# brson/synth2

Measured on AMD Instinct MI355X. Metric: voice-samples/sec (mono) at 64k voices per GPU, 48 kHz, 1024-frame buffers, higher is better.
Workload: dtype f32

## Files before the change

include/s2r.h:

```cpp
#ifndef S2R_H
#define S2R_H
#include <stddef.h>
#include <stdint.h>

#ifdef __cplusplus
extern "C" {
#endif

#define S2R_ABI_VERSION 4

typedef enum {
    S2R_OK = 0,
    S2R_ERR_INVALID = -1,
    S2R_ERR_NO_DEVICE = -2,
    S2R_ERR_HIP = -3,
    S2R_ERR_PATCH_SYNTAX = -4,
    S2R_ERR_PATCH_RANGE = -5,
    S2R_ERR_TOO_MANY_FRAMES = -6,
    S2R_ERR_OFFSET_OVERFLOW = -7,
    S2R_ERR_OUT_OF_MEMORY = -8
} s2r_status;

typedef enum { S2R_OSC_SQUARE = 0, S2R_OSC_SAW = 1, S2R_OSC_TRIANGLE = 2, S2R_OSC_SINE = 3,
               S2R_OSC_DPW_SAW = 4, S2R_OSC_DPW_SQUARE = 5, S2R_OSC_DPW_TRIANGLE = 6 } s2r_osc_kind;
// ... 197 lines not shown

typedef void (*s2r_voice_log_fn)(void *user, uint32_t voice_index, uint8_t note);
int s2r_set_voice_log(s2r_synth *s, s2r_voice_log_fn fn, void *user);

uint32_t s2r_abi_version(void);
const char *s2r_build_id(void);
uint32_t s2r_shard_voices(const s2r_synth *s);
uint32_t s2r_block_voices(const s2r_synth *s);
uint32_t s2r_device_count(const s2r_synth *s);
uint64_t s2r_double_release_count(const s2r_synth *s);
int s2r_set_low_latency(s2r_synth *s, int enabled);
int s2r_low_latency_active(const s2r_synth *s);
#define S2R_EXCHANGE_HANDLE_BYTES 64
int s2r_exchange_create(s2r_synth *s, uint32_t n_ranks, void *handle_out, size_t handle_bytes);
int s2r_exchange_attach(s2r_synth *s, uint32_t rank, uint32_t n_ranks, const void *handle, size_t handle_bytes);
int s2r_set_resident(s2r_synth *s, int enabled);
int s2r_resident_active(const s2r_synth *s);
int s2r_quiesce(s2r_synth *s);
int s2r_set_timing(s2r_synth *s, int enabled);
int s2r_set_flat_shortcut(s2r_synth *s, int enabled);
int s2r_set_coeff_stream(s2r_synth *s, int enabled);
int s2r_set_uniform_window(s2r_synth *s, int enabled);
int s2r_uniform_window_chunks(s2r_synth *s, uint64_t *chunks);
float s2r_last_render_ms(s2r_synth *s);
const char *s2r_last_error(const s2r_synth *s);
const char *s2r_status_string(int status);


#define S2R_STREAM_CHARS_PER_SAMPLE 18u
#define S2R_STREAM_FRAMES 4096u
#define S2R_STREAM_RATE_HZ 32000u
size_t s2r_stream_frame_json(const float *samples, size_t n, char *out, size_t cap);

int s2r_parse_patch_text(const char *text, size_t len, s2r_patch *out, char *err_buf, size_t err_cap);

float s2r_voice_pan(float pan, float key_spread, uint8_t note);
void s2r_pan_gains(float p, float *gl, float *gr);

float s2r_voice_gain(float level, float velocity_sens, float velocity);

void s2r_fader_gains(float pan, float w, float fader, float pan_shift, float *gl, float *gr);

float s2r_send_gain(float g, float send);

typedef struct s2r_voice_pool s2r_voice_pool;
s2r_voice_pool *s2r_voice_pool_create(uint32_t total_voices);
// ... 14 lines not shown
```

synth2_amd/csrc/s2r_device.h:

```cpp
#pragma once
#include <hip/hip_runtime_api.h>
#include <stdint.h>
#include "s2r.h"

#define S2R_VF_STARTED 1u
#define S2R_VF_RELEASED 2u

struct S2rEnv {
    float A;
    float D;
    float S;
    float R;
    float sus_off;
    float slope_att;
    float slope_dec;
    float slope_rel;
};

struct S2rVoiceArrays {
    float *pitch;
    uint32_t *offset;
    uint32_t *release;
    uint32_t *flags;
    float *phase;
// ... 76 lines not shown
    int32_t fast_div_sr;
    int32_t no_flat_shortcut;
    uint32_t frames;
    uint32_t n_voices;
    uint32_t frames_stride;
    uint32_t super_frames;
    S2rVoiceArrays v;
    float *block_partials;
    float *direct_out;
    int32_t direct_stereo;
    S2rDone done;
    float *per_voice;
    const float *sin_table;
    const float *noise_tab;
    S2rTabRef tab;
    const S2rTimedEvent *tev;
    int32_t *voice_ev_head;
    unsigned long long *stamps;
    unsigned long long *timeline;
    uint32_t tl_slot;
    uint32_t uw_frames;
    const S2rBankEntry *bank;
    uint32_t bank_size;
    const uint32_t *ov_heads_counter;
    uint32_t ov_heads_target;
    uint32_t *ov_render_counter;
    uint32_t *ov_fail;
    const S2rTimedEvent *tev_src;
    S2rTimedEvent *tev_copy;
    const uint32_t *slices;
    uint32_t *arrive;
    uint32_t arrive_target;
    S2rMixTail mt;
    uint32_t *uw_count;
};
#define S2R_UW_FRAMES 1024u
#define S2R_UW_PLANES 4u
#define S2R_UW_MIN_RUN 3u

struct S2rVoiceEvent {
    uint32_t voice;
    uint32_t flags;
    float pitch;
    uint32_t seed;
};
#define S2R_EV_RESTART 1u
#define S2R_EV_RELEASE 2u
#define S2R_EV_PROGRAM_SHIFT 16

struct S2rTimedEvent {
    uint32_t voice;
    uint32_t frame;
    uint32_t flags;
    float pitch;
    uint32_t seed;
    int32_t next;
    uint32_t program;
    uint32_t _pad;
// ... 210 lines not shown
```

synth2_amd/csrc/s2r_host.cpp:

```cpp
#include <hip/hip_runtime.h>
#include <algorithm>
#include <cmath>
#include <cstdarg>
#include <cstdio>
#include <cstdlib>
#include <cstring>
#include <ctime>
#include <atomic>
#include <memory>
#include <new>
#include <string>
#include <vector>

#include "s2r.h"
#include "s2r_device.h"
#include "s2r_math.h"
#include "s2r_patch.h"
#include "s2r_post.h"
#include "s2r_rules.h"
#include "s2r_voices.h"

namespace {

constexpr int kEventSlots = 4;
// ... 211 lines not shown
        }
    } mixer;
    unsigned gains_dirty = kGainsAll;
    float *gains_host = nullptr, *gains_dev = nullptr;
    hipEvent_t gains_sent = nullptr;
    float *pan_rows = nullptr;
    uint32_t pan_slice = 0;
    float *pan_partials = nullptr;
    std::vector<hipEvent_t> pan_ev;
    size_t pan_ev_used = 0;
    float pan_mix_ms = -1.0f;
    char *bus_gains_host = nullptr, *bus_gains_dev = nullptr;
    hipEvent_t bus_gains_sent = nullptr;
    float *bus_partials = nullptr;
    float *bus_out = nullptr, *bus_out_dev = nullptr;
    float bus_mix_ms = -1.0f;
    bool bus_dev_ramped = false;
    S2rPostChain post;
    float pitch_table[256];
    hipEvent_t t0 = nullptr, t1 = nullptr;
    bool timing = false, timed = false, no_flat_shortcut = false;
    uint64_t double_release = 0;
    bool uniform_window = true;
    uint32_t *uw_count_dev = nullptr;
    s2r_voice_log_fn voice_log = nullptr;
    void *voice_log_user = nullptr;
    bool broken = false;
    std::string err = "";
};


namespace {

int set_err(s2r_synth *s, int code, const char *fmt, ...) {
    if (s) {
        char buf[512];
        va_list ap; va_start(ap, fmt); vsnprintf(buf, sizeof buf, fmt, ap); va_end(ap);
        s->err = buf;
    }
    return code;
}

#define S2R_TRY(call) do { const int rc_t_ = (call); if (rc_t_ != S2R_OK) return rc_t_; } while (0)
#define S2R_QUIESCE(s) S2R_TRY(quiesce(s))
int resident_stop(s2r_synth *s);
int pool_stop(s2r_synth *s);
// ... 278 lines not shown
    p.noise_level = s->bank[0].noise;
    p.lpf_freq = s->bank[0].lpf_freq;
    p.amt_osc = s->bank[0].mod_env_to_osc_freq;
    p.amt_lpf = s->bank[0].mod_env_to_lpf_freq;
    p.lpf_kind = s->bank[0].lpf_kind;
    p.lpf_damping = s->bank[0].lpf_kind >= S2R_FILT_BP2 ? s->bank[0].lpf_q : s->bank[0].lpf_damping;
    p.amp = resolve_env(s->bank[0].amp_env, sample_rate);
    p.mod = resolve_env(s->bank[0].mod_env, sample_rate);
    p.sr = (float)sample_rate;
    p.rcp_sr = 1.0f / p.sr;
    p.fast_div_sr = (fast_div_rate(sample_rate) && s->bank[0].lpf_freq >= 0x1p-30f && s->bank[0].lpf_freq <= 0x1p30f) ? 1 : 0;
    p.no_flat_shortcut = s->no_flat_shortcut ? 1 : 0;
    p.frames = (uint32_t)frames;
    p.n_voices = s->shard_voices;
    p.frames_stride = partials_stride(s->cfg.max_frames);
    p.v = s->v;
    p.block_partials = s->block_partials;
    p.per_voice = nullptr;
    p.sin_table = s->sin_dev;
    { static const bool off = [] { const char *e = std::getenv("S2R_NOISE_TAB"); return e && e[0] == '0'; }();
      p.noise_tab = off ? nullptr : s->noise_dev; }
    p.bank = s->bank_dev;
    p.bank_size = (uint32_t)s->bank.size();
    p.uw_count = s->uniform_window ? s->uw_count_dev : nullptr;
    return p;
}

int ensure_bank(s2r_synth *s, uint32_t sample_rate, hipStream_t stream, bool *bank_kernel_out) {
    bool bank_kernel = s->bank.size() > 1;
    for (const s2r_patch &pt : s->bank) if (pt.osc_kind > S2R_OSC_SINE) bank_kernel = true;
    if (bank_kernel && (s->bank_dirty || s->bank_rate != sample_rate)) {
        std::vector<S2rBankEntry> host(s->bank.size());
        std::vector<S2rTabBuild> builds(s->bank.size());
        size_t tab_floats = 0;
        const float srf = (float)sample_rate;
        for (size_t k = 0; k < s->bank.size(); k++) {
            const s2r_patch &pt = s->bank[k];
            S2rBankEntry &e = host[k];
            std::memset(&e, 0, sizeof e);
            e.osc_kind = pt.osc_kind; e.osc_gain = pt.osc_gain; e.noise_level = pt.noise; e.lpf_freq = pt.lpf_freq;
            e.amt_osc = pt.mod_env_to_osc_freq; e.amt_lpf = pt.mod_env_to_lpf_freq; e.lpf_kind = pt.lpf_kind;
            e.lpf_shape = pt.lpf_kind >= S2R_FILT_BP2 ? pt.lpf_q : pt.lpf_damping;
            e.amp = resolve_env(pt.amp_env, sample_rate);
            e.mod = resolve_env(pt.mod_env, sample_rate);
            S2rTabBuild &b = builds[k];
            b = S2rTabBuild{};
            if (s->use_tab && !s->no_flat_shortcut && plan_tables(e.mod, b) && tab_floats + (size_t)b.plane * 4u <= ((size_t)1 << 28)) {
// ... 1246 lines not shown
            CREATE_HIP(hipMalloc((void **)&s->partials2[1], (size_t)s->n_blocks * partials_stride(cfg->max_frames) * sizeof(float)));
            CREATE_HIP(hipMalloc((void **)&s->heads2[1], pv * sizeof(int32_t)));
            CREATE_HIP(hipMemsetAsync(s->heads2[1], 0xff, pv * sizeof(int32_t), s->stream));
            CREATE_HIP(hipMalloc((void **)&s->tevcopy2[1], (size_t)s->tev_capacity * sizeof(S2rTimedEvent)));
            CREATE_HIP(hipMalloc((void **)&s->ov_words, sizeof(S2rOverlapWords)));
            CREATE_HIP(hipMemsetAsync(s->ov_words, 0, sizeof(S2rOverlapWords), s->stream));
            s->ov_enabled = true;
        }
    }
    CREATE_HIP(hipEventCreate(&s->t0));
    CREATE_HIP(hipEventCreate(&s->t1));
    {
        float table[1024];
        build_sin_table(table);
        if (crc32_bytes(table, sizeof table) != kSinTableCrc) {
            fprintf(stderr, "libs2r: regenerated SIN_TABLE does not match the reference table (CRC mismatch)\n");
            release_all(s);
            return S2R_ERR_INVALID;
        }
        CREATE_HIP(hipMalloc((void **)&s->sin_dev, sizeof table));
        CREATE_HIP(hipMemcpy(s->sin_dev, table, sizeof table, hipMemcpyHostToDevice));
        CREATE_HIP(hipMalloc((void **)&s->noise_dev, 65536 * sizeof(float)));
        CREATE_HIP(s2r_launch_noise_table(s->noise_dev, s->stream));
        CREATE_HIP(hipMalloc((void **)&s->uw_count_dev, sizeof(uint32_t)));
        CREATE_HIP(hipMemsetAsync(s->uw_count_dev, 0, sizeof(uint32_t), s->stream));
    }
    CREATE_HIP(hipStreamSynchronize(s->stream));
#undef CREATE_HIP
    *out = s;
    return S2R_OK;
}


int s2r_create(const s2r_config *cfg, s2r_synth **out) {
    if (!cfg || !out || cfg->struct_size != sizeof(s2r_config)) return S2R_ERR_INVALID;
    *out = nullptr;
    if (cfg->n_devices <= 1) {
        s2r_config one = *cfg;
        if (cfg->n_devices == 1) one.device = cfg->devices[0];
        one.n_devices = 0;
        return create_single(&one, nullptr, nullptr, out);
    }
    const uint32_t n = cfg->n_devices;
    const uint32_t bv = cfg->block_voices ? cfg->block_voices : 256u;
    if (n > S2R_MAX_DEVICES || cfg->total_voices == 0 || cfg->max_frames == 0 || cfg->reserved0 != 0) return S2R_ERR_INVALID;
    if (cfg->shard_begin || cfg->shard_voices || cfg->shard_index || cfg->shard_count > 1 || cfg->mix_groups > 1) return S2R_ERR_INVALID;
    if (bv < 64 || bv > 1024 || (bv & 63u) || cfg->total_voices % ((uint64_t)n * bv)) return S2R_ERR_INVALID;
    if (cfg->shard_interleave && ((cfg->shard_interleave & 15u) || bv % cfg->shard_interleave)) return S2R_ERR_INVALID;
// ... 1099 lines not shown
}

uint32_t s2r_shard_voices(const s2r_synth *s) { return s ? s->shard_voices : 0; }
uint32_t s2r_block_voices(const s2r_synth *s) { return s ? s->block_voices : 0; }
uint32_t s2r_device_count(const s2r_synth *s) { return s ? (s->kids.empty() ? 1u : (uint32_t)s->kids.size()) : 0; }
uint64_t s2r_double_release_count(const s2r_synth *s) { return s ? s->double_release : 0; }

int s2r_set_flat_shortcut(s2r_synth *s, int enabled) {
    if (!s) return S2R_ERR_INVALID;
    S2R_QUIESCE(s);
    s->no_flat_shortcut = enabled == 0;
    for (s2r_synth *kid : s->kids) kid->no_flat_shortcut = s->no_flat_shortcut;
    return S2R_OK;
}

int s2r_set_uniform_window(s2r_synth *s, int enabled) {
    if (!s) return S2R_ERR_INVALID;
    S2R_QUIESCE(s);
    s->uniform_window = enabled != 0;
    for (s2r_synth *kid : s->kids) kid->uniform_window = s->uniform_window;
    return S2R_OK;
}

int s2r_uniform_window_chunks(s2r_synth *s, uint64_t *chunks) {
    if (!s || !chunks) return S2R_ERR_INVALID;
    S2R_QUIESCE(s);
    uint64_t total = 0;
    auto one = [&](s2r_synth *h) -> int {
        if (!h->uw_count_dev) return S2R_OK;
        uint32_t n = 0;
        S2R_HIP(s, hipSetDevice(h->device));
        S2R_HIP(s, hipDeviceSynchronize());
        S2R_HIP(s, hipMemcpy(&n, h->uw_count_dev, sizeof n, hipMemcpyDeviceToHost));
        total += n;
        return S2R_OK;
    };
    if (s->kids.empty()) { S2R_TRY(one(s)); }
    else for (s2r_synth *kid : s->kids) { S2R_TRY(one(kid)); }
    *chunks = total;
    return S2R_OK;
}

int s2r_set_coeff_stream(s2r_synth *s, int enabled) {
    if (!s) return S2R_ERR_INVALID;
    S2R_QUIESCE(s);
    s->use_tab = enabled != 0;
    s->use_arg_events = enabled != 2 && enabled != 4;
    s->bank_dirty = true;
    for (s2r_synth *kid : s->kids) { kid->use_tab = s->use_tab; kid->use_arg_events = s->use_arg_events; kid->bank_dirty = true; }
    return S2R_OK;
}

int s2r_set_low_latency(s2r_synth *s, int enabled) {
    if (!s) return S2R_ERR_INVALID;
    if (s->parent || !s->kids.empty()) return set_err(s, S2R_ERR_INVALID, "s2r_set_low_latency takes a single-device handle");
    S2R_QUIESCE(s);
    if (enabled && !s->res_host) {
        S2R_HIP(s, hipSetDevice(s->device));
        S2R_HIP(s, hipHostMalloc((void **)&s->res_host, 64 * sizeof(uint32_t), kHostPolled));
        std::memset(s->res_host, 0, 64 * sizeof(uint32_t));
        S2R_HIP(s, hipHostGetDevicePointer((void **)&s->res_dev, s->res_host, 0));
        s->res_cmd = s->res_host; s->res_cmd_dev = s->res_dev; s->res_cmd_vram = false;
        S2R_HIP(s, hipHostMalloc((void **)&s->res_gran, S2R_RES_GRANULE_FRAMES * sizeof(unsigned long long), kHostPolled));
        std::memset(s->res_gran, 0, S2R_RES_GRANULE_FRAMES * sizeof(unsigned long long));
// ... 205 lines not shown
```

synth2_amd/csrc/s2r_render_onepole.inc:

```
#include "s2r_kern_common.h"

namespace {

template <int OSC, bool FM, int MODE, int MAXT, bool UWK = false>
__device__ __forceinline__ void render_fill(const S2rRenderArgs &a, const FillCtl &ctl) {
    const S2rRenderParams &p = a.p;
    constexpr bool PV = MODE == 1;
    constexpr bool TEV = MODE == 2;
    const uint32_t kSuper = p.super_frames;
    __shared__ uint64_t sT[S2R_EXP2F_N];
    __shared__ __attribute__((aligned(8))) float sSin[OSC == S2R_OSC_SINE ? 2048 : 2];
    extern __shared__ __attribute__((aligned(16))) float s_dyn[];
    __shared__ uint32_t s_word;

    const uint32_t tid = threadIdx.x;
    const uint32_t lane = tid & 63u, wave = tid >> 6, n_waves = blockDim.x >> 6;
    constexpr uint32_t VW = 64;
    constexpr uint32_t GW = VW / 16;
    const uint32_t n_groups = n_waves * GW;
    float *const sW = s_dyn;
    constexpr uint32_t kTile = kChunk * kTileRow;
    const uint32_t sw_floats = s2r_sw_buffers(p.frames, kSuper) * n_groups * kSuper;
    float *const tile = s_dyn + sw_floats + wave * kTile;
    float *const wave_scratch = s_dyn + sw_floats + n_waves * kTile + wave * (64u + (UWK ? S2R_UW_PLANES * p.uw_frames : 0u));
    uint32_t uw_chunks = 0;
    const uint32_t tile_lds = (uint32_t)__builtin_amdgcn_readfirstlane((int)(uint32_t)(uintptr_t)tile);
    const uint32_t vi = blockIdx.x * blockDim.x + tid;
#if defined(S2R_STAMPS)
    uint32_t stamp_k = 0;
    auto stamp = [&](uint32_t slot) { if (p.stamps && lane == 0 && slot < 16u) p.stamps[(size_t)(vi >> 6) * 16u + slot] = __builtin_amdgcn_s_memtime(); };
    stamp(0);
#else
    auto stamp = [&](uint32_t) {};
    uint32_t stamp_k = 0; (void)stamp_k;
#endif
    uint32_t dbg_events = 0, dbg_dense = 0, dbg_general = 0, dbg_runs = 0, dbg_runchunks = 0;
    unsigned long long dbg_t_dense = 0, dbg_t_run = 0;
    unsigned long long dbg_t_top = 0, dbg_t_sel = 0; (void)dbg_t_top; (void)dbg_t_sel;
    unsigned long long dbg_t_pick1 = 0, dbg_t_casc = 0; (void)dbg_t_pick1; (void)dbg_t_casc;
    (void)dbg_events; (void)dbg_dense; (void)dbg_general; (void)dbg_runs; (void)dbg_runchunks; (void)dbg_t_dense; (void)dbg_t_run;
#if defined(S2R_STAMPS)
#define S2R_DBG_NOW() __builtin_amdgcn_s_memtime()
#else
#define S2R_DBG_NOW() 0ull
#endif

    tl_mark(p.timeline, p.tl_slot, 0);
    if (tid < S2R_EXP2F_N) sT[tid] = c_exp2f_table[tid];
    if (OSC == S2R_OSC_SINE)
        for (uint32_t i = tid; i < 1024u; i += blockDim.x) { sSin[2u * i] = p.sin_table[(i + 1023u) & 1023u]; sSin[2u * i + 1u] = p.sin_table[i]; }

    apply_arg_events(p, ctl.n_events, ctl.ev, vi, lane);

    const bool in_range = vi < p.n_voices;
    const bool ovh = TEV && (ctl.fused || ctl.ov_heads_counter != nullptr);
    if (TEV && ctl.fused) { fused_heads(ctl); stamp(7); }
    else if (ovh) {
        if (tid == 0) { const bool ok = ov_wait(ctl.ov_heads_counter, ctl.ov_heads_target); if (!ok) ov_raise(ctl.fail, 1u); s_word = ok ? 1u : 0u; }
        __syncthreads();
        if (s_word == 0u) {
            float *row = ctl.partials + (size_t)blockIdx.x * p.frames_stride;
            for (uint32_t f = 4u * tid; f < p.frames_stride && f < ((ctl.frames + 3u) & ~3u); f += 4u * blockDim.x) ov_store4(row + f, (f4){0.0f, 0.0f, 0.0f, 0.0f});
// ... 51 lines not shown
        while (ev_idx >= 0 && !(ev_next.flags & S2R_EV_RESTART)) {
            const uint32_t rel = r.offset + ev_next.frame;
            const bool base_ok = r.offset <= (1u << 24) || r.offset >= 0u - ctl.frames;
            if (!(base_ok && rel <= (1u << 24))) break;
            if ((ev_next.flags & S2R_EV_RELEASE) && live && !r.released) {
                r.released = true;
                r.release_u = rel;
                took_release = true;
            }
            ev_dirty = true;
            ev_idx = ev_next.next;
            ev_frame = 0xffffffffu;
            if (ev_idx >= 0) { ev_next = tev_at(ev_idx); ev_frame = ev_next.frame; }
        }
    };
    if (TEV) take_releases();
    r.seed_rot = (seed << 5) | (seed >> 27);

    const float rel_f = r.released ? (float)r.release_u : 4294967296.0f;
    r.ro_a = __builtin_fmaxf(rel_f, p.amp.sus_off); r.end_a = r.ro_a + p.amp.R;
    r.ro_m = __builtin_fmaxf(rel_f, p.mod.sus_off); r.end_m = r.ro_m + p.mod.R;

    OscK k_const = make_osck<OSC>(p.sr / (1.0f * r.pitch));
    uint32_t seed_now = seed;

    EnvRun ea = env_stage_at(p.amp, r.ro_a, r.end_a, (float)r.offset);
    EnvRun em = env_stage_at(p.mod, r.ro_m, r.end_m, (float)r.offset);
    float thr_min = __builtin_fminf(ea.s3, em.s3);
    FlatCache fc;
    fc.xc = 0.0f; fc.k = k_const;

    __syncthreads();
    const bool have_tab = p.tab.base != nullptr && !p.no_flat_shortcut;
    FlatConsts fcc = (have_tab && (!FM || p.tab.fm_plane != 0u)) ? flat_consts_from_tables<OSC, FM>(p, r.pitch) : make_flat_consts<OSC, FM>(p, r.pitch, sT);
    fc = refresh_flat<OSC, FM>(fcc, em, fc);

    const bool wave_live = __ballot(live || ev_idx >= 0) != 0ull;
    bool wave_events = TEV && __ballot(ev_idx >= 0) != 0ull;
    const uint32_t x16_frames = ctl.frames & ~(uint32_t)(kChunk - 1);
    const bool fast_ok = __ballot(!(r.phase >= 0.0f && r.phase < 1.0f)) == 0ull &&
        (FM || __ballot(!(k_const.period >= 0x1p-126f && k_const.period < __builtin_inff())) == 0ull);
    const size_t pv_base = (size_t)vi * ctl.frames;
    float *bp = ctl.partials + (size_t)blockIdx.x * p.frames_stride;
    uint32_t buf = 0;

    auto reduce_chunk = [&](uint32_t f_base, uint32_t n_frames) {
        const uint32_t f = lane & 15u, grp = lane >> 4;
// ... 23 lines not shown
        w_aflat = __ballot(live && ea.s0 != 0.0f) == 0ull;
        classify_uniform();
    };
    auto reclassify = [&]() {
        reclassify_stages();
        w_aligned = p.noise_tab != nullptr && __ballot(((r.offset | r.seed_rot) & 15u) != 0u) == 0ull;
        w_small = __ballot(r.offset + ctl.frames > (1u << 24)) == 0ull;
    };
    reclassify();
    stamp(1);

    auto apply_events_lane = [&](uint32_t fpos) -> bool {
        bool restarted = false, released_now = false;
        took_release = false;
        while (ev_frame == fpos) {
            const S2rTimedEvent e = ev_next;
            if (e.flags & S2R_EV_RESTART) {
                r.pitch = e.pitch;
                r.offset = 0u - fpos;
                r.release_u = 0u;
                r.released = (e.flags & S2R_EV_RELEASE) != 0u;
                r.phase = 0.0f; r.last = 0.0f;
                const S2rTimedEvent er = tev_at(ev_idx);
                seed_now = er.seed;
                r.seed_rot = (seed_now << 5) | (seed_now >> 27);
                program_now = er.program;
                live = true; ev_restart = true; restarted = true;
                k_const = make_osck<OSC>(p.sr / (1.0f * r.pitch));
            } else if ((e.flags & S2R_EV_RELEASE) && live && !r.released) {
                r.released = true;
                r.release_u = r.offset + fpos;
                released_now = true;
            }
            ev_dirty = true;
            ev_idx = e.next;
            ev_frame = 0xffffffffu;
            if (ev_idx >= 0) { ev_next = tev_at(ev_idx); ev_frame = ev_next.frame; }
            take_releases();
        }
        const float rf = r.released ? (float)r.release_u : 4294967296.0f;
        r.ro_a = __builtin_fmaxf(rf, p.amp.sus_off); r.end_a = r.ro_a + p.amp.R;
        r.ro_m = __builtin_fmaxf(rf, p.mod.sus_off); r.end_m = r.ro_m + p.mod.R;
        const float t0 = (float)(r.offset + fpos);
        if (restarted) {
            if (FM) {
                const FlatConsts n = (have_tab && p.tab.fm_plane != 0u) ? flat_consts_from_tables<OSC, FM>(p, r.pitch) : make_flat_consts<OSC, FM>(p, r.pitch, sT);
                fcc.k_s = n.k_s; fcc.k_0 = n.k_0;
            }
// ... 141 lines not shown
                            const bool hit = ev_frame == fnext;
                            if (__ballot((hit && !plain) || !((float)(onext + (kChunk - 1u)) < thr_min)) != 0ull) break;
                            pend_rel = hit ? onext : pend_rel;
                            ev_frame = hit ? 0xffffffffu : ev_frame;
                            if ((c16 & 0x30u) == 0x30u) {
                                const uint64_t pending = __ballot(ev_frame != 0xffffffffu);
                                if (pending == 0ull) { idle_exit = true; break; }
                                if (__builtin_popcountll(pending) <= 4) {
                                    const uint32_t nxt = wave_min_u32(ev_frame);
                                    if (((nxt - fnext) >> 4) > 8u) { idle_exit = true; break; }
                                }
                            }
                        }
                    }
                    commit_plain();
                    wave_events = __ballot(ev_idx >= 0) != 0ull;
                    dense_stay = wave_events && !idle_exit && !inside && c16 >= n_x16;
                    dbg_t_dense += S2R_DBG_NOW() - dbg_td0;
                    reclassify();
                    if (c16 >= n_x16) break;
                    if (!inside) { c16 -= kChunk; continue; }
                }
                const unsigned long long dbg_ts0 = S2R_DBG_NOW();
                const uint32_t o_chunk = r.offset + sc0 + c16;
                if (fast_ok) {
                    const uint32_t left = (n_x16 - c16) / kChunk;
                    auto clear_for = [&](uint32_t n) {
                        bool bad = !((float)(o_chunk + n * kChunk - 1u) < thr_min);
                        if (TEV) bad = bad || ev_frame < sc0 + c16 + n * kChunk;
                        return __ballot(bad) == 0ull;
                    };
                    auto pick_run = [&]() -> uint32_t {
                        const float q = ((thr_min - (float)o_chunk) + 1.0f) * 0.0625f;
                        float nf = __builtin_ceilf(q) - 1.0f;
                        nf = __builtin_fminf(__builtin_fmaxf(nf, 0.0f), (float)left);
                        uint32_t n = (uint32_t)nf;
                        if (TEV) { const uint32_t ne = (ev_frame - (sc0 + c16)) >> 4; n = ne < n ? ne : n; }
                        n = wave_min_u32(n);
                        if (n == 0u) return 0u;
                        if (clear_for(n)) return n;
                        return (n > 1u && clear_for(1u)) ? 1u : 0u;
                    };
                    {
                        const float t0 = (float)o_chunk;
                        if (__ballot(!(t0 < thr_min)) != 0ull) {
                            end_of_release(t0);
                            thr_min = __builtin_fminf(ea.s3, em.s3);
                            if (!(t0 < thr_min)) {
                                ea = env_stage_at(p.amp, r.ro_a, r.end_a, t0);
                                em = env_stage_at(p.mod, r.ro_m, r.end_m, t0);
                                thr_min = __builtin_fminf(ea.s3, em.s3);
                            }
                            fc = refresh_flat<OSC, FM>(fcc, em, fc);
                            reclassify_stages();
                        }
                    }
                    const unsigned long long dbg_ts1 = S2R_DBG_NOW();
                    dbg_t_casc += dbg_ts1 - dbg_ts0;
                    uint32_t run = pick_run();
                    dbg_t_pick1 += S2R_DBG_NOW() - dbg_ts1;
                    bool flat = false, tab_ok = false, offs_small = false;
                    if (run) {
                        run = (uint32_t)__builtin_amdgcn_readfirstlane((int)run);
                        offs_small = w_small || __ballot(o_chunk + run * kChunk > (1u << 24)) == 0ull;
                        flat = w_flat;
                        tab_ok = !flat && have_tab && offs_small;
                        if (FM && !flat && !tab_ok) run = 0;
                        if (FM && !flat && __ballot(live && !(p.sr >= r.pitch * 0x1p-115f)) != 0ull) run = 0;
                    }
                    if (run) {
                        ++dbg_runs; dbg_runchunks += run;
                        const unsigned long long dbg_tr0 = S2R_DBG_NOW();
                        dbg_t_sel += dbg_tr0 - dbg_ts0;
                        float *const sw_row = sW + (buf * n_groups + wave * GW + rgrp) * kSuper + rf;
                        const TabCur cur = tab_cursor(p.tab, em.s4, r.ro_m > p.mod.sus_off, r.release_u, live);
                        auto run_chunks = [&](auto src_tag, auto nz_tag, auto aflat_tag, auto uw_tag) {
                            constexpr int SRC = decltype(src_tag)::value;
                            constexpr int NZ = decltype(nz_tag)::value;
                            constexpr bool AFLAT = decltype(aflat_tag)::value;
                            constexpr bool UW = decltype(uw_tag)::value;
                            if (UW) {
                                const uint32_t o_run = (uint32_t)__builtin_amdgcn_readfirstlane((int)o_chunk);
                                uw_fill(p, ea, r.seed_rot, o_run, run, p.tab.base + (ptrdiff_t)(cur.idx + (int32_t)o_chunk), wave_scratch + 64u, lane);
                                uw_chunks += run;
                            }
                            for (uint32_t i = 0; i < run; ++i) {
                                const uint32_t f0 = c16 + i * kChunk;
                                *pend_dst = tsum();
                                float *pvd = (PV && in_range) ? p.per_voice + pv_base + sc0 + f0 : nullptr;
                                const uint32_t oc = o_chunk + i * kChunk;
                                const float *tp = p.tab.base + (ptrdiff_t)(cur.idx + (int32_t)(oc & cur.mask));
                                chunk_fast<OSC, SRC, 0, (FM && SRC == 1), NZ, AFLAT, UW>(p, r, ea, em, fc, FM ? fc.k : k_const, oc, tp, sT, sSin, live,
                                                                              tile_lds, pvd, nullptr, nullptr, wave_scratch + 64u + i * kChunk);
                                __builtin_amdgcn_wave_barrier();
                                pend_dst = sw_row + f0;
                            }
                        };
                        const bool small = p.noise_level == 0.0f && offs_small;
                        const bool aligned = small && w_aligned && ((sc0 + c16) & 15u) == 0u;
                        const bool aflat = aligned && w_aflat;
                        using T = std::true_type; using F = std::false_type;
                        using N0 = std::integral_constant<int, 0>; using N1 = std::integral_constant<int, 1>; using N2 = std::integral_constant<int, 2>;
                        using UWon = std::integral_constant<bool, UWK && !FM>;
                        const bool uw = UWon::value && w_uni && run >= S2R_UW_MIN_RUN;
                        if (tab_ok) {
                            if (aflat) run_chunks(N1{}, N2{}, T{}, F{});
                            else if (aligned && uw) run_chunks(N1{}, N2{}, F{}, UWon{});
                            else if (aligned) run_chunks(N1{}, N2{}, F{}, F{});
                            else if (small) run_chunks(N1{}, N1{}, F{}, F{});
                            else run_chunks(N1{}, N0{}, F{}, F{});
                        } else if (flat) {
                            if (aflat) run_chunks(N0{}, N2{}, T{}, F{});
                            else if (aligned) run_chunks(N0{}, N2{}, F{}, F{});
                            else if (small) run_chunks(N0{}, N1{}, F{}, F{});
                            else run_chunks(N0{}, N0{}, F{}, F{});
                        } else if (!FM) {
                            if (aligned) run_chunks(N2{}, N2{}, F{}, F{});
                            else if (small) run_chunks(N2{}, N1{}, F{}, F{});
                            else run_chunks(N2{}, N0{}, F{}, F{});
// ... 41 lines not shown
            }
        } else {
            for (uint32_t i = lane; i < GW * kSuper; i += 64u)
                sW[(buf * n_groups + wave * GW + i / kSuper) * kSuper + (i % kSuper)] = 0.0f;
            if (PV) { if (in_range) for (uint32_t i = 0; i < n_sc; ++i) p.per_voice[pv_base + sc0 + i] = 0.0f; }
        }
        stamp(2u + 2u * stamp_k);
        __syncthreads();
        combine_groups(p, ctl.done, sW + (size_t)buf * n_groups * kSuper, n_groups, kSuper, n_sc, sc0, bp + sc0, tid, blockDim.x, ctl.granules, ctl.granule_tag, ctl.fused || ctl.ov_render_counter != nullptr);
        buf ^= 1u;
        stamp(3u + 2u * stamp_k);
        ++stamp_k;
    }

    if (live) {
        const uint32_t o = r.offset;
        p.v.offset[vi] = (!ev_dirty && o > 0xffffffffu - ctl.frames) ? 0xffffffffu : o + ctl.frames;
        p.v.phase[vi] = r.phase;
        p.v.lpf_last[vi] = r.last;
        if (ev_dirty) {
            p.v.pitch[vi] = r.pitch;
            p.v.release[vi] = r.release_u;
            p.v.flags[vi] = S2R_VF_STARTED | (r.released ? S2R_VF_RELEASED : 0u);
            p.v.seed[vi] = seed_now;
            if (ev_restart) {
                p.v.fx1[vi] = 0.0f; p.v.fx2[vi] = 0.0f; p.v.fy1[vi] = 0.0f; p.v.fy2[vi] = 0.0f;
                p.v.osc_z[vi] = s2r_u2f(S2R_OSC_Z_NONE);
                p.v.program[vi] = program_now;
            }
        }
    }
    if (UWK && uw_chunks != 0u && lane == 0u) __hip_atomic_fetch_add(p.uw_count, uw_chunks, __ATOMIC_RELAXED, __HIP_MEMORY_SCOPE_AGENT);
    if (p.direct_out && ctl.granules == nullptr) signal_done(ctl.done, 1u);
    if (ctl.ov_render_counter != nullptr) ov_signal(ctl.ov_render_counter);
#if defined(S2R_STAMPS)
    if (p.stamps && lane == 0) p.stamps[(size_t)(vi >> 6) * 16u + 8u] = __builtin_amdgcn_s_memrealtime();
    if (ctl.fused) fused_tail(p, ctl, sW, &s_word, p.stamps ? p.stamps + (size_t)(vi >> 6) * 16u : nullptr);
#else
    if (ctl.fused) fused_tail(p, ctl, sW, &s_word);
#endif
#if defined(S2R_STAMPS)
    if (p.stamps && lane == 0) { unsigned long long *d = p.stamps + (size_t)(vi >> 6) * 16u; d[11] = dbg_events; d[12] = (unsigned long long)dbg_dense | ((dbg_t_pick1 & 0x3fffffull) << 20) | ((dbg_t_casc & 0x3fffffull) << 42); d[13] = (dbg_t_top << 32) | (dbg_t_sel & 0xffffffffull); d[14] = dbg_runs;
        d[10] = ((unsigned long long)dbg_runchunks << 48) | ((dbg_t_dense & 0xffffffull) << 24) | (dbg_t_run & 0xffffffull); }
#endif
    stamp(15);
    tl_mark(p.timeline, p.tl_slot, 1);
}

template <int OSC, bool FM, int MODE, int MAXT>
__global__ void __launch_bounds__(MAXT, (MAXT == 256 ? 2 : 1)) s2r_render_kernel(const S2rRenderArgs a) {
    const FillCtl ctl = fill_ctl_from_args(a);
    render_fill<OSC, FM, MODE, MAXT, MAXT == 256>(a, ctl);
}

template <int OSC, bool FM>
__global__ void __launch_bounds__(256, 1) s2r_resident_kernel(const S2rRenderArgs a, const S2rResident rs) {
    __shared__ uint32_t s_cmd[S2R_RES_CMD_WORDS];
    const uint32_t tid = threadIdx.x, lane = tid & 63u;
    uint32_t last = rs.first_seq - 1u;
    for (;;) {
        if (tid < 64u) {
            const unsigned long long t0 = __builtin_amdgcn_s_memrealtime();
            uint32_t polls = 0;
            for (;;) {
                uint32_t w = 0u;
// ... 22 lines not shown
        ctl.granules = ctl.frames <= S2R_RES_GRANULE_FRAMES ? rs.granules : nullptr;
        ctl.granule_tag = s_cmd[3];
        if (ctl.frames != 0u && ctl.frames <= a.p.frames) render_fill<OSC, FM, 0, 256>(a, ctl);
        __syncthreads();
    }
    if (tid == 0u) __hip_atomic_store(rs.exited, rs.launch_id, __ATOMIC_RELAXED, __HIP_MEMORY_SCOPE_SYSTEM);
}

template <int OSC, bool FM>
__global__ void __launch_bounds__(256, 1) s2r_pool_kernel(const S2rRenderArgs a, const S2rPool pl) {
    pool_loop(a, pl, [&](const FillCtl &ctl) __attribute__((always_inline)) { render_fill<OSC, FM, 2, 256>(a, ctl); });
}

template <int OSC, bool FM, int MODE>
hipError_t launch_mode(const S2rRenderArgs &a0, uint32_t block_voices, hipStream_t stream) {
    static thread_local S2rRenderArgs a;
    a = a0;
    S2rRenderParams &p = a.p;
    const uint32_t grid = (p.n_voices + block_voices - 1) / block_voices;
    const uint32_t n_waves = block_voices / 64, n_groups = n_waves * 4;
    p.super_frames = s2r_pick_super_frames(n_groups, grid, p.frames);
    size_t lds = sizeof(float) * ((size_t)s2r_sw_buffers(p.frames, p.super_frames) * n_groups * p.super_frames + (size_t)n_waves * (kChunk * kTileRow + 64));
    p.uw_frames = 0u;
    if (p.uw_count != nullptr && !FM && block_voices <= 256 && p.super_frames == kSuperWhole && s2r_sw_buffers(p.frames, p.super_frames) == 1u) {
        const size_t with_uw = lds + sizeof(float) * (size_t)n_waves * S2R_UW_PLANES * S2R_UW_FRAMES;
        if (with_uw + 8192u + 8u * S2R_EXP2F_N + 64u <= 160u * 1024u) { lds = with_uw; p.uw_frames = S2R_UW_FRAMES; }
    }
    if (lds > 65536) {
        static thread_local size_t told256 = 0, told1024 = 0;
        if (block_voices <= 256 && told256 < lds) {
            const hipError_t e = hipFuncSetAttribute((const void *)s2r_render_kernel<OSC, FM, MODE, 256>, hipFuncAttributeMaxDynamicSharedMemorySize, (int)lds);
            if (e != hipSuccess) return e;
            told256 = lds;
        } else if (block_voices > 256 && told1024 < lds) {
            const hipError_t e = hipFuncSetAttribute((const void *)s2r_render_kernel<OSC, FM, MODE, 1024>, hipFuncAttributeMaxDynamicSharedMemorySize, (int)lds);
            if (e != hipSuccess) return e;
            told1024 = lds;
        }
    }
    if (block_voices <= 256) hipLaunchKernelGGL((s2r_render_kernel<OSC, FM, MODE, 256>), dim3(grid), dim3(block_voices), lds, stream, a);
    else hipLaunchKernelGGL((s2r_render_kernel<OSC, FM, MODE, 1024>), dim3(grid), dim3(block_voices), lds, stream, a);
    return hipGetLastError();
}

template <int OSC, bool FM>
hipError_t launch_resident(const S2rRenderArgs &a0, const S2rResident &rs, uint32_t block_voices, hipStream_t stream) {
    static thread_local S2rRenderArgs a;
// ... 66 lines not shown
```

synth2_amd/synth.py:

```python
import ctypes as C
import os

import numpy as np

from . import build as _build

OSC_SQUARE, OSC_SAW, OSC_TRIANGLE, OSC_SINE = 0, 1, 2, 3
OSC_DPW_SAW, OSC_DPW_SQUARE, OSC_DPW_TRIANGLE = 4, 5, 6

S2R_OK = 0
S2R_ERR_INVALID = -1
S2R_ERR_NO_DEVICE = -2
S2R_ERR_HIP = -3
S2R_ERR_PATCH_SYNTAX = -4
S2R_ERR_PATCH_RANGE = -5
S2R_ERR_TOO_MANY_FRAMES = -6
S2R_ERR_OFFSET_OVERFLOW = -7
S2R_ERR_OUT_OF_MEMORY = -8
MAX_BUSES = 8
MAX_IR_TAPS = 65536
MAX_DELAY_FRAMES = 262144
CHORUS_MAX_VOICES = 8
CHORUS_MAX_DELAY = 4095.0
IR_SEGMENT = 256
# ... 188 lines not shown
        "s2r_sum_partials_device": (C.c_int, [C.c_void_p, C.c_uint32, C.c_size_t, C.c_void_p, C.c_void_p]),
        "s2r_render_voices": (C.c_int, [H, _f32p, C.c_size_t, C.c_uint32]),
        "s2r_process_layers": (C.c_int, [H, C.c_void_p, C.c_uint32, _f32p, C.c_size_t, C.c_uint32]),
        "s2r_set_voice_log": (C.c_int, [H, VOICE_LOG_FN, C.c_void_p]),
        "s2r_export_state": (C.c_int, [H, C.c_void_p]),
        "s2r_import_state": (C.c_int, [H, C.c_void_p]),
        "s2r_set_noise_seed": (C.c_int, [H, C.c_uint32, C.c_uint32]),
        "s2r_shard_voices": (C.c_uint32, [H]),
        "s2r_block_voices": (C.c_uint32, [H]),
        "s2r_device_count": (C.c_uint32, [H]),
        "s2r_double_release_count": (C.c_uint64, [H]),
        "s2r_set_timing": (C.c_int, [H, C.c_int]),
        "s2r_set_low_latency": (C.c_int, [H, C.c_int]),
        "s2r_low_latency_active": (C.c_int, [H]),
        "s2r_set_resident": (C.c_int, [H, C.c_int]),
        "s2r_resident_active": (C.c_int, [H]),
        "s2r_quiesce": (C.c_int, [H]),
        "s2r_exchange_create": (C.c_int, [H, C.c_uint32, C.c_void_p, C.c_size_t]),
        "s2r_exchange_attach": (C.c_int, [H, C.c_uint32, C.c_uint32, C.c_void_p, C.c_size_t]),
        "s2r_set_flat_shortcut": (C.c_int, [H, C.c_int]),
        "s2r_set_coeff_stream": (C.c_int, [H, C.c_int]),
        "s2r_set_uniform_window": (C.c_int, [H, C.c_int]),
        "s2r_uniform_window_chunks": (C.c_int, [H, C.POINTER(C.c_uint64)]),
        "s2r_last_render_ms": (C.c_float, [H]),
        "s2r_last_error": (C.c_char_p, [H]),
        "s2r_parse_patch_text": (C.c_int, [C.c_char_p, C.c_size_t, C.POINTER(Patch), C.c_char_p, C.c_size_t]),
        "s2r_voice_pool_create": (H, [C.c_uint32]),
        "s2r_voice_pool_destroy": (None, [H]),
        "s2r_voice_pool_note_on": (C.c_uint32, [H, C.c_uint8, C.c_float]),
        "s2r_voice_pool_note_off": (C.c_int64, [H, C.c_uint8]),
        "s2r_voice_pool_advance": (None, [H, C.c_uint64]),
        "s2r_voice_pool_next_voice": (C.c_uint32, [H]),
        "s2r_voice_pool_set_threads": (None, [H, C.c_uint32, C.c_size_t]),
        "s2r_voice_pool_resolve": (C.c_uint32, [H, C.c_void_p, C.c_size_t, C.c_uint32, C.c_void_p]),
        "s2r_voice_pool_query": (C.c_int, [H, C.c_uint32, C.POINTER(VoiceState)]),
    }
    for name, (res, args) in sig.items():
        if _build.AB_LIB and not hasattr(L, name):
            continue
        f = getattr(L, name)
        f.restype = res
        f.argtypes = args
    L._fill_raw = C.CFUNCTYPE(C.c_int, H, C.c_void_p, C.c_size_t, C.c_uint32)(("s2r_fill", L))
    _lib = L
    return L

# ... 588 lines not shown

    def import_state(self, arr):
        arr = np.ascontiguousarray(arr, dtype=VOICE_STATE_DTYPE)
        assert arr.size == self.shard_voices
        self._check(self.L.s2r_import_state(self.h, arr.ctypes.data))

    def set_noise_seed(self, voice_index, seed):
        self._check(self.L.s2r_set_noise_seed(self.h, voice_index, seed))

    def set_flat_shortcut(self, enabled=True):
        self._check(self.L.s2r_set_flat_shortcut(self.h, 1 if enabled else 0))

    def set_coeff_stream(self, enabled=True):
        self._check(self.L.s2r_set_coeff_stream(self.h, int(enabled)))

    def set_uniform_window(self, enabled=True):
        self._check(self.L.s2r_set_uniform_window(self.h, 1 if enabled else 0))

    def uniform_window_chunks(self):
        n = C.c_uint64(0)
        self._check(self.L.s2r_uniform_window_chunks(self.h, C.byref(n)))
        return int(n.value)

    def set_low_latency(self, enabled=True):
        self._check(self.L.s2r_set_low_latency(self.h, 1 if enabled else 0))

    @property
    def low_latency_active(self):
        return bool(self.L.s2r_low_latency_active(self.h))

    def set_resident(self, enabled=True):
        self._check(self.L.s2r_set_resident(self.h, 1 if enabled else 0))

    @property
    def resident_active(self):
        return bool(self.L.s2r_resident_active(self.h))

    def quiesce(self):
        self._check(self.L.s2r_quiesce(self.h))

    def exchange_create(self, n_ranks):
        buf = C.create_string_buffer(64)
        self._check(self.L.s2r_exchange_create(self.h, n_ranks, buf, 64))
        return buf.raw

    def exchange_attach(self, rank, n_ranks, handle):
# ... 16 lines not shown
```

Measured before the change: 1708 billion.

## Chain consecutive fast runs in place instead of returning to the outer loop

```diff
diff --git a/include/s2r.h b/include/s2r.h
--- a/include/s2r.h
+++ b/include/s2r.h
@@ -243,6 +243,8 @@
 int s2r_set_coeff_stream(s2r_synth *s, int enabled);
 int s2r_set_uniform_window(s2r_synth *s, int enabled);
 int s2r_uniform_window_chunks(s2r_synth *s, uint64_t *chunks);
+int s2r_set_turns_in_place(s2r_synth *s, int enabled);
+int s2r_turns_in_place(s2r_synth *s, uint64_t *turns);
 float s2r_last_render_ms(s2r_synth *s);
 const char *s2r_last_error(const s2r_synth *s);
 const char *s2r_status_string(int status);
diff --git a/synth2_amd/csrc/s2r_device.h b/synth2_amd/csrc/s2r_device.h
--- a/synth2_amd/csrc/s2r_device.h
+++ b/synth2_amd/csrc/s2r_device.h
@@ -122,6 +122,7 @@
     uint32_t uw_frames;
     const S2rBankEntry *bank;
     uint32_t bank_size;
+    uint32_t paths;
     const uint32_t *ov_heads_counter;
     uint32_t ov_heads_target;
     uint32_t *ov_render_counter;
@@ -132,8 +133,10 @@
     uint32_t *arrive;
     uint32_t arrive_target;
     S2rMixTail mt;
-    uint32_t *uw_count;
-};
+    uint32_t *path_counts;
+};
+#define S2R_PATH_UW 1u
+#define S2R_PATH_TIP 2u
 #define S2R_UW_FRAMES 1024u
 #define S2R_UW_PLANES 4u
 #define S2R_UW_MIN_RUN 3u
diff --git a/synth2_amd/csrc/s2r_host.cpp b/synth2_amd/csrc/s2r_host.cpp
--- a/synth2_amd/csrc/s2r_host.cpp
+++ b/synth2_amd/csrc/s2r_host.cpp
@@ -257,6 +257,7 @@
     bool timing = false, timed = false, no_flat_shortcut = false;
     uint64_t double_release = 0;
     bool uniform_window = true;
+    bool turns_in_place = true;
     uint32_t *uw_count_dev = nullptr;
     s2r_voice_log_fn voice_log = nullptr;
     void *voice_log_user = nullptr;
@@ -581,7 +582,8 @@
       p.noise_tab = off ? nullptr : s->noise_dev; }
     p.bank = s->bank_dev;
     p.bank_size = (uint32_t)s->bank.size();
-    p.uw_count = s->uniform_window ? s->uw_count_dev : nullptr;
+    p.path_counts = s->uw_count_dev;
+    p.paths = !s->uw_count_dev ? 0u : (s->uniform_window ? S2R_PATH_UW : 0u) | (s->turns_in_place ? S2R_PATH_TIP : 0u);
     return p;
 }
 
@@ -1874,8 +1876,8 @@
         CREATE_HIP(hipMemcpy(s->sin_dev, table, sizeof table, hipMemcpyHostToDevice));
         CREATE_HIP(hipMalloc((void **)&s->noise_dev, 65536 * sizeof(float)));
         CREATE_HIP(s2r_launch_noise_table(s->noise_dev, s->stream));
-        CREATE_HIP(hipMalloc((void **)&s->uw_count_dev, sizeof(uint32_t)));
-        CREATE_HIP(hipMemsetAsync(s->uw_count_dev, 0, sizeof(uint32_t), s->stream));
+        CREATE_HIP(hipMalloc((void **)&s->uw_count_dev, 2 * sizeof(uint32_t)));
+        CREATE_HIP(hipMemsetAsync(s->uw_count_dev, 0, 2 * sizeof(uint32_t), s->stream));
     }
     CREATE_HIP(hipStreamSynchronize(s->stream));
 #undef CREATE_HIP
@@ -3021,8 +3023,8 @@
     return S2R_OK;
 }
 
-int s2r_uniform_window_chunks(s2r_synth *s, uint64_t *chunks) {
-    if (!s || !chunks) return S2R_ERR_INVALID;
+static int read_path_count(s2r_synth *s, uint32_t which, uint64_t *count) {
+    if (!s || !count) return S2R_ERR_INVALID;
     S2R_QUIESCE(s);
     uint64_t total = 0;
     auto one = [&](s2r_synth *h) -> int {
@@ -3030,15 +3032,27 @@
         uint32_t n = 0;
         S2R_HIP(s, hipSetDevice(h->device));
         S2R_HIP(s, hipDeviceSynchronize());
-        S2R_HIP(s, hipMemcpy(&n, h->uw_count_dev, sizeof n, hipMemcpyDeviceToHost));
+        S2R_HIP(s, hipMemcpy(&n, h->uw_count_dev + which, sizeof n, hipMemcpyDeviceToHost));
         total += n;
         return S2R_OK;
     };
     if (s->kids.empty()) { S2R_TRY(one(s)); }
     else for (s2r_synth *kid : s->kids) { S2R_TRY(one(kid)); }
-    *chunks = total;
-    return S2R_OK;
-}
+    *count = total;
+    return S2R_OK;
+}
+
+int s2r_uniform_window_chunks(s2r_synth *s, uint64_t *chunks) { return read_path_count(s, 0u, chunks); }
+
+int s2r_set_turns_in_place(s2r_synth *s, int enabled) {
+    if (!s) return S2R_ERR_INVALID;
+    S2R_QUIESCE(s);
+    s->turns_in_place = enabled != 0;
+    for (s2r_synth *kid : s->kids) kid->turns_in_place = s->turns_in_place;
+    return S2R_OK;
+}
+
+int s2r_turns_in_place(s2r_synth *s, uint64_t *turns) { return read_path_count(s, 1u, turns); }
 
 int s2r_set_coeff_stream(s2r_synth *s, int enabled) {
     if (!s) return S2R_ERR_INVALID;
diff --git a/synth2_amd/csrc/s2r_render_onepole.inc b/synth2_amd/csrc/s2r_render_onepole.inc
--- a/synth2_amd/csrc/s2r_render_onepole.inc
+++ b/synth2_amd/csrc/s2r_render_onepole.inc
@@ -34,10 +34,11 @@
     auto stamp = [&](uint32_t) {};
     uint32_t stamp_k = 0; (void)stamp_k;
 #endif
-    uint32_t dbg_events = 0, dbg_dense = 0, dbg_general = 0, dbg_runs = 0, dbg_runchunks = 0;
+    uint32_t dbg_events = 0, dbg_dense = 0, dbg_general = 0, dbg_runs = 0, dbg_runchunks = 0, dbg_turns = 0; (void)dbg_turns;
     unsigned long long dbg_t_dense = 0, dbg_t_run = 0;
     unsigned long long dbg_t_top = 0, dbg_t_sel = 0; (void)dbg_t_top; (void)dbg_t_sel;
     unsigned long long dbg_t_pick1 = 0, dbg_t_casc = 0; (void)dbg_t_pick1; (void)dbg_t_casc;
+    unsigned long long dbg_t_tip = 0; (void)dbg_t_tip;
     (void)dbg_events; (void)dbg_dense; (void)dbg_general; (void)dbg_runs; (void)dbg_runchunks; (void)dbg_t_dense; (void)dbg_t_run;
 #if defined(S2R_STAMPS)
 #define S2R_DBG_NOW() __builtin_amdgcn_s_memtime()
@@ -135,7 +136,6 @@
     r.ro_m = __builtin_fmaxf(rel_f, p.mod.sus_off); r.end_m = r.ro_m + p.mod.R;
 
     OscK k_const = make_osck<OSC>(p.sr / (1.0f * r.pitch));
-    uint32_t seed_now = seed;
 
     EnvRun ea = env_stage_at(p.amp, r.ro_a, r.end_a, (float)r.offset);
     EnvRun em = env_stage_at(p.mod, r.ro_m, r.end_m, (float)r.offset);
@@ -205,8 +205,7 @@
                 r.released = (e.flags & S2R_EV_RELEASE) != 0u;
                 r.phase = 0.0f; r.last = 0.0f;
                 const S2rTimedEvent er = tev_at(ev_idx);
-                seed_now = er.seed;
-                r.seed_rot = (seed_now << 5) | (seed_now >> 27);
+                r.seed_rot = (er.seed << 5) | (er.seed >> 27);
                 program_now = er.program;
                 live = true; ev_restart = true; restarted = true;
                 k_const = make_osck<OSC>(p.sr / (1.0f * r.pitch));
@@ -394,18 +393,18 @@
                     if (!inside) { c16 -= kChunk; continue; }
                 }
                 const unsigned long long dbg_ts0 = S2R_DBG_NOW();
-                const uint32_t o_chunk = r.offset + sc0 + c16;
+                auto o_chunk = [&]() -> uint32_t { return r.offset + (sc0 + c16); };
                 if (fast_ok) {
-                    const uint32_t left = (n_x16 - c16) / kChunk;
+                    auto left = [&]() -> uint32_t { return (n_x16 - c16) / kChunk; };
                     auto clear_for = [&](uint32_t n) {
-                        bool bad = !((float)(o_chunk + n * kChunk - 1u) < thr_min);
+                        bool bad = !((float)(o_chunk() + n * kChunk - 1u) < thr_min);
                         if (TEV) bad = bad || ev_frame < sc0 + c16 + n * kChunk;
                         return __ballot(bad) == 0ull;
                     };
                     auto pick_run = [&]() -> uint32_t {
-                        const float q = ((thr_min - (float)o_chunk) + 1.0f) * 0.0625f;
+                        const float q = ((thr_min - (float)o_chunk()) + 1.0f) * 0.0625f;
                         float nf = __builtin_ceilf(q) - 1.0f;
-                        nf = __builtin_fminf(__builtin_fmaxf(nf, 0.0f), (float)left);
+                        nf = __builtin_fminf(__builtin_fmaxf(nf, 0.0f), (float)left());
                         uint32_t n = (uint32_t)nf;
                         if (TEV) { const uint32_t ne = (ev_frame - (sc0 + c16)) >> 4; n = ne < n ? ne : n; }
                         n = wave_min_u32(n);
@@ -414,7 +413,7 @@
                         return (n > 1u && clear_for(1u)) ? 1u : 0u;
                     };
                     {
-                        const float t0 = (float)o_chunk;
+                        const float t0 = (float)o_chunk();
                         if (__ballot(!(t0 < thr_min)) != 0ull) {
                             end_of_release(t0);
                             thr_min = __builtin_fminf(ea.s3, em.s3);
@@ -434,7 +433,7 @@
                     bool flat = false, tab_ok = false, offs_small = false;
                     if (run) {
                         run = (uint32_t)__builtin_amdgcn_readfirstlane((int)run);
-                        offs_small = w_small || __ballot(o_chunk + run * kChunk > (1u << 24)) == 0ull;
+                        offs_small = w_small || __ballot(o_chunk() + run * kChunk > (1u << 24)) == 0ull;
                         flat = w_flat;
                         tab_ok = !flat && have_tab && offs_small;
                         if (FM && !flat && !tab_ok) run = 0;
@@ -452,21 +451,43 @@
                             constexpr bool AFLAT = decltype(aflat_tag)::value;
                             constexpr bool UW = decltype(uw_tag)::value;
                             if (UW) {
-                                const uint32_t o_run = (uint32_t)__builtin_amdgcn_readfirstlane((int)o_chunk);
-                                uw_fill(p, ea, r.seed_rot, o_run, run, p.tab.base + (ptrdiff_t)(cur.idx + (int32_t)o_chunk), wave_scratch + 64u, lane);
+                                const uint32_t o_run = (uint32_t)__builtin_amdgcn_readfirstlane((int)o_chunk());
+                                uw_fill(p, ea, r.seed_rot, o_run, run, p.tab.base + (ptrdiff_t)(cur.idx + (int32_t)o_chunk()), wave_scratch + 64u, lane);
                                 uw_chunks += run;
                             }
+                            constexpr bool TIP = UWK && !FM && SRC == 0 && NZ == 2 && !AFLAT && !UW;
+                            uint32_t turns = 0;
+                            for (;;) {
                             for (uint32_t i = 0; i < run; ++i) {
                                 const uint32_t f0 = c16 + i * kChunk;
                                 *pend_dst = tsum();
                                 float *pvd = (PV && in_range) ? p.per_voice + pv_base + sc0 + f0 : nullptr;
-                                const uint32_t oc = o_chunk + i * kChunk;
+                                const uint32_t oc = o_chunk() + i * kChunk;
                                 const float *tp = p.tab.base + (ptrdiff_t)(cur.idx + (int32_t)(oc & cur.mask));
                                 chunk_fast<OSC, SRC, 0, (FM && SRC == 1), NZ, AFLAT, UW>(p, r, ea, em, fc, FM ? fc.k : k_const, oc, tp, sT, sSin, live,
                                                                               tile_lds, pvd, nullptr, nullptr, wave_scratch + 64u + i * kChunk);
                                 __builtin_amdgcn_wave_barrier();
                                 pend_dst = sw_row + f0;
                             }
+                            if (!TIP || (p.paths & S2R_PATH_TIP) == 0u || !w_small || left() == run) break;
+                            const unsigned long long dbg_tp0 = S2R_DBG_NOW();
+                            const uint32_t step = run * kChunk;
+                            const float t0 = (float)(o_chunk() + step);
+                            end_of_release(t0);
+                            thr_min = __builtin_fminf(ea.s3, em.s3);
+                            fc = refresh_flat<OSC, FM>(fcc, em, fc);
+                            bool out = !(t0 < thr_min) || (live && em.s0 != 0.0f);
+                            if (TEV) out = out || ev_frame - (sc0 + c16 + step) < 3u * kChunk;
+                            if (__ballot(out) != 0ull) { dbg_t_tip += S2R_DBG_NOW() - dbg_tp0; break; }
+                            c16 += step;
+                            const uint32_t next = pick_run();
+                            dbg_t_tip += S2R_DBG_NOW() - dbg_tp0;
+                            if (next == 0u) { c16 -= step; break; }
+                            run = (uint32_t)__builtin_amdgcn_readfirstlane((int)next);
+                            ++dbg_runs; dbg_runchunks += run; ++turns; ++dbg_turns;
+                            }
+                            if (TIP && (p.paths & S2R_PATH_TIP) != 0u && w_small) reclassify_stages();
+                            if (TIP && turns != 0u && lane == 0u) __hip_atomic_fetch_add(p.path_counts + 1, turns, __ATOMIC_RELAXED, __HIP_MEMORY_SCOPE_AGENT);
                         };
                         const bool small = p.noise_level == 0.0f && offs_small;
                         const bool aligned = small && w_aligned && ((sc0 + c16) & 15u) == 0u;
@@ -554,7 +575,7 @@
             p.v.pitch[vi] = r.pitch;
             p.v.release[vi] = r.release_u;
             p.v.flags[vi] = S2R_VF_STARTED | (r.released ? S2R_VF_RELEASED : 0u);
-            p.v.seed[vi] = seed_now;
+            p.v.seed[vi] = (r.seed_rot >> 5) | (r.seed_rot << 27);
             if (ev_restart) {
                 p.v.fx1[vi] = 0.0f; p.v.fx2[vi] = 0.0f; p.v.fy1[vi] = 0.0f; p.v.fy2[vi] = 0.0f;
                 p.v.osc_z[vi] = s2r_u2f(S2R_OSC_Z_NONE);
@@ -562,7 +583,7 @@
             }
         }
     }
-    if (UWK && uw_chunks != 0u && lane == 0u) __hip_atomic_fetch_add(p.uw_count, uw_chunks, __ATOMIC_RELAXED, __HIP_MEMORY_SCOPE_AGENT);
+    if (UWK && uw_chunks != 0u && lane == 0u) __hip_atomic_fetch_add(p.path_counts, uw_chunks, __ATOMIC_RELAXED, __HIP_MEMORY_SCOPE_AGENT);
     if (p.direct_out && ctl.granules == nullptr) signal_done(ctl.done, 1u);
     if (ctl.ov_render_counter != nullptr) ov_signal(ctl.ov_render_counter);
 #if defined(S2R_STAMPS)
@@ -572,7 +593,7 @@
     if (ctl.fused) fused_tail(p, ctl, sW, &s_word);
 #endif
 #if defined(S2R_STAMPS)
-    if (p.stamps && lane == 0) { unsigned long long *d = p.stamps + (size_t)(vi >> 6) * 16u; d[11] = dbg_events; d[12] = (unsigned long long)dbg_dense | ((dbg_t_pick1 & 0x3fffffull) << 20) | ((dbg_t_casc & 0x3fffffull) << 42); d[13] = (dbg_t_top << 32) | (dbg_t_sel & 0xffffffffull); d[14] = dbg_runs;
+    if (p.stamps && lane == 0) { unsigned long long *d = p.stamps + (size_t)(vi >> 6) * 16u; d[11] = (unsigned long long)dbg_events | (dbg_t_tip << 32); d[12] = (unsigned long long)dbg_dense | ((dbg_t_pick1 & 0x3fffffull) << 20) | ((dbg_t_casc & 0x3fffffull) << 42); d[13] = (dbg_t_top << 32) | (dbg_t_sel & 0xffffffffull); d[14] = (unsigned long long)dbg_runs | ((unsigned long long)dbg_turns << 32);
         d[10] = ((unsigned long long)dbg_runchunks << 48) | ((dbg_t_dense & 0xffffffull) << 24) | (dbg_t_run & 0xffffffull); }
 #endif
     stamp(15);
@@ -641,7 +662,7 @@
     p.super_frames = s2r_pick_super_frames(n_groups, grid, p.frames);
     size_t lds = sizeof(float) * ((size_t)s2r_sw_buffers(p.frames, p.super_frames) * n_groups * p.super_frames + (size_t)n_waves * (kChunk * kTileRow + 64));
     p.uw_frames = 0u;
-    if (p.uw_count != nullptr && !FM && block_voices <= 256 && p.super_frames == kSuperWhole && s2r_sw_buffers(p.frames, p.super_frames) == 1u) {
+    if ((p.paths & S2R_PATH_UW) != 0u && !FM && block_voices <= 256 && p.super_frames == kSuperWhole && s2r_sw_buffers(p.frames, p.super_frames) == 1u) {
         const size_t with_uw = lds + sizeof(float) * (size_t)n_waves * S2R_UW_PLANES * S2R_UW_FRAMES;
         if (with_uw + 8192u + 8u * S2R_EXP2F_N + 64u <= 160u * 1024u) { lds = with_uw; p.uw_frames = S2R_UW_FRAMES; }
     }
diff --git a/synth2_amd/synth.py b/synth2_amd/synth.py
--- a/synth2_amd/synth.py
+++ b/synth2_amd/synth.py
@@ -234,6 +234,8 @@
         "s2r_set_coeff_stream": (C.c_int, [H, C.c_int]),
         "s2r_set_uniform_window": (C.c_int, [H, C.c_int]),
         "s2r_uniform_window_chunks": (C.c_int, [H, C.POINTER(C.c_uint64)]),
+        "s2r_set_turns_in_place": (C.c_int, [H, C.c_int]),
+        "s2r_turns_in_place": (C.c_int, [H, C.POINTER(C.c_uint64)]),
         "s2r_last_render_ms": (C.c_float, [H]),
         "s2r_last_error": (C.c_char_p, [H]),
         "s2r_parse_patch_text": (C.c_int, [C.c_char_p, C.c_size_t, C.POINTER(Patch), C.c_char_p, C.c_size_t]),
@@ -868,6 +870,14 @@
         self._check(self.L.s2r_uniform_window_chunks(self.h, C.byref(n)))
         return int(n.value)
 
+    def set_turns_in_place(self, enabled=True):
+        self._check(self.L.s2r_set_turns_in_place(self.h, 1 if enabled else 0))
+
+    def turns_in_place(self):
+        n = C.c_uint64(0)
+        self._check(self.L.s2r_turns_in_place(self.h, C.byref(n)))
+        return int(n.value)
+
     def set_low_latency(self, enabled=True):
         self._check(self.L.s2r_set_low_latency(self.h, 1 if enabled else 0))
 
```

Result: no change. 1717 billion (median of 3 runs) (+0.5%).
